# PJLab-ADG/DetZero

Hardware: AMD Instinct MI355X
Metric: LiDAR frames/sec (160k pts, 0.1m voxels) (higher is better)
Workload: dtype f32 as f16 pairs (hi+lo, 22-bit significand; 3 f16 MFMA per product, f32 accumulate)

## Files before the change

detzero_amd/centerpoint.py:

```python
import contextlib
import math
import os

import numpy as np
import torch
import torch.nn as nn

from . import det_modules as cp_modules
from . import iou3d_nms_utils, ops, range_audit as _range_audit
from .lib import DetZeroHipError
from .range_audit import RangeAudit


class CenterPoint(nn.Module):
    def __init__(self, model_cfg, num_class, dataset):
        super().__init__()
        self.model_cfg = model_cfg
        self.num_class = num_class
        self.dataset = dataset
        self.tta = getattr(self.dataset, 'tta', False)
        self.class_names = dataset.class_names
        self.register_buffer('global_step', torch.LongTensor(1).zero_())
        self.second_stage = model_cfg.SECOND_STAGE
        self.module_list = self.build_networks()
# ... 288 lines not shown
        self.split_min = int(os.environ.get('DZ_TUNE_SPLIT_MIN', '12'))
        self._subs = None
        self._way_streams = None
        self.side_key = 0
        self.fork_ok = True
        self.info = dataset_info
        self.mode = mode
        self.dynamic = dynamic
        self.head = model.dense_head
        if len(self.head.class_names_each_head) != 1:
            raise DetZeroHipError('FramePipeline: the batched route packs ONE head\'s detections (the layout of every DetZero config); a '
                                  'multi-head CenterHead runs through the module API (CenterPoint.forward)')
        post = self.head.model_cfg.POST_PROCESSING
        self.k = post.MAX_OBJ_PER_SAMPLE
        self.post_max = post.NMS_CONFIG.NMS_POST_MAXSIZE
        self._streams = {}
        self.level_caps = None
        self._ws = {}
        self.dense_group = int(os.environ.get('DZ_TUNE_DENSE_GROUP', '16'))
        self.last_overflow = None
        self._overflow_acc = None
        self.head_at_candidates = True
        self._partial_head = None

    def _voxelize(self, frames, cid=0):
        info = self.info
        rng = info.point_cloud_range
        nb = len(frames)
        if self.dynamic:
            pb = torch.cat([torch.cat([p.new_full((p.shape[0], 1), float(i)), p], dim=1) for i, p in enumerate(frames)], dim=0)
            return ops.voxelize_dynamic_nosync(pb.contiguous(), rng, info.voxel_size, nb, xy_range_mask=True)
        dev = frames[0].device
        main = torch.cuda.current_stream(dev)
        cap = int(min(info.max_voxels[self.mode], max(max(p.shape[0] for p in frames), 1)))
        c = frames[0].shape[1]
        if nb > 1 and all(p.shape[0] == frames[0].shape[0] for p in frames):
            if isinstance(frames, _StackedFrames):
                pts = frames.tensor.reshape(-1, c)
            else:
                pts = torch.cat(list(frames), dim=0)
            feats, coords, _ = ops.voxelize_hard_mean_batched(pts, nb, rng, info.voxel_size, info.max_points_per_voxel,
                                                              info.max_voxels[self.mode], cap, xy_range_mask=True)
            return feats, coords, None
        feats = torch.empty((nb * cap, c), dtype=torch.float32, device=dev)
        coords = torch.full((nb * cap, 4), -1, dtype=torch.int32, device=dev)
        d_ns = torch.zeros((nb,), dtype=torch.int32, device=dev)
# ... 114 lines not shown
            if self._overflow_acc is None:
                if torch.cuda.is_current_stream_capturing():
                    raise DetZeroHipError('FramePipeline: the overflow counter must exist before graph capture - run calibrate() or '
                                          'one eager pass first (a counter allocated inside a capture is re-zeroed by every replay)')
                self._overflow_acc = torch.zeros((), dtype=torch.int32, device=self.last_overflow.device)
            self._overflow_acc |= self.last_overflow.to(torch.int32)
        return res

    @torch.no_grad()
    def dense_stage(self, res, nb):
        with self._recording():
            return self._dense_stage(res, nb)

    def _dense_stage(self, res, nb):
        m = self.model
        x, lvl = res['encoded']
        sparse = m.backbone3d.math != 0 and m.backbone2d.math == m.backbone3d.math and m.backbone2d.sparse_input_ok(x.shape[1], lvl.shape[0])
        if sparse:
            bev = ops.bev_row_index(lvl, x.shape[0], pad=1)
            run2d = lambda g0, ng: m.backbone2d.run(None, ng, sparse_in=(x, bev[g0:g0 + ng]))
        else:
            bev = ops.sparse_to_bev(x, lvl, x.shape[1], pad=1, math=m.backbone3d.math)
            run2d = lambda g0, ng: m.backbone2d.run(bev[g0:g0 + ng], ng)
        per_frame = bev.shape[1] * bev.shape[2] * max(int(m.backbone2d.num_bev_features), 2 * int(x.shape[1])) * 4
        group = max(1, min(self.dense_group if self.dense_group > 0 else nb, (2 ** 31 - 1) // per_frame))
        at_cand = self.head_at_candidates and self.head.at_candidates_ok()
        self._partial_head = None
        if at_cand:
            self.head.candidate_params()
        if nb <= group:
            with cp_modules.workspace(self._ws):
                concat = run2d(0, nb)
                if not at_cand:
                    return self.head.run_convs(concat, nb)
                shared = self.head.run_shared(concat, nb)
                hd, hh, hw_ = self.head.run_score_head(shared, nb)
                self._partial_head = (hd.data_ptr(), tuple(hd.shape), shared)
                return hd, hh, hw_
        st = {'out': None, 'h': 0, 'w': 0, 'shared': None}

        def head_of_group(concat, g0, ng):
            if at_cand:
                if st['shared'] is None:
                    st['shared'] = cp_modules.bordered_zeros('head.shared_all', (nb,) + tuple(concat.shape[1:3]) + (self.head.plan()['c'],), concat.device)
                hd, st['h'], st['w'] = self.head.run_score_head(self.head.run_shared(concat, ng, out=st['shared'][g0:g0 + ng]), ng)
            else:
                hd, st['h'], st['w'] = self.head.run_convs(concat, ng)
            if st['out'] is None:
                st['out'] = hd.new_empty((nb,) + tuple(hd.shape[1:]))
# ... 256 lines not shown
```

detzero_amd/csrc/conv2d_h.hip:

```cpp
#include "hgemm.h"

namespace dz {

int conv3x3_h_variant(const dz_conv2d_desc &p);
int conv3x3_h_launch(const dz_conv2d_desc &p, int bc, int math, int out_f32, size_t w_bytes, hipStream_t stream);

template <class T, class M, bool OUT_F32, int NS>
__global__ __launch_bounds__(256) void k_conv2d_h(dz_conv2d_desc p, long m_total, unsigned int in_bytes, unsigned int w_bytes) {
    extern __shared__ __attribute__((aligned(16))) unsigned char smem_raw[];
    v4u *const smem = reinterpret_cast<v4u *>(smem_raw);
    __shared__ int in_pix[T::BP];
    __shared__ int out_pix[T::BP];
    __shared__ __attribute__((aligned(16))) float sc_s[T::BC], sh_s[T::BC];

    const int tid = threadIdx.x, lane = tid & 63, wid = tid >> 6;
    const int wp = wid / T::WC, wc = wid % T::WC;
    const int ntn = p.cout_pad / T::BC;
    const int nty = ntn * p.groups;
    const int nwg = gridDim.x, q8 = nwg >> 3, r8 = nwg & 7, xcd = blockIdx.x & 7;
    const int lid = (xcd < r8 ? xcd * (q8 + 1) : r8 * (q8 + 1) + (xcd - r8) * q8) + (blockIdx.x >> 3);
    const int by = lid % nty;
    const int grp = by / ntn;
    const int n0 = (by % ntn) * T::BC;
    const long row0 = (long)(lid / nty) * T::BP;
// ... 157 lines not shown
#pragma unroll
                    for (int e = 0; e < 4; ++e)
                        if (col + e < gcout) o[e] = v[e];
                } else {
                    uint2 hi, lo;
                    split4<M>(v, hi, lo);
                    unsigned char *g = reinterpret_cast<unsigned char *>(p.out) +
                                       ((size_t)op * p.out_cstride + ooff + (col & ~7)) * 4 + (col & 7) * 2;
                    *reinterpret_cast<uint2 *>(g) = hi;
                    *reinterpret_cast<uint2 *>(g + 16) = lo;
                }
            }
        }
    }
}

template <class T, class M, bool OUT_F32, int NS>
static int launch_conv_h(const dz_conv2d_desc &p, size_t w_bytes, hipStream_t stream) {
    const long m_total = (long)p.batch * p.ho * p.wo;
    dim3 grid(ceil_div(m_total, T::BP) * (p.cout_pad / T::BC) * p.groups);
    const size_t in_bytes = (size_t)p.batch * p.in_hp * p.in_wp * p.in_cstride * sizeof(float);
    if (in_bytes >= 0x80000000ull || w_bytes >= 0x80000000ull) {
        set_error("dz_conv2d_forward_split: image of %zu bytes / weights of %zu bytes exceed the 2 GiB buffer-addressing limit", in_bytes, w_bytes);
        return DZ_ERR_UNSUPPORTED;
    }
    static PerDeviceFlags lds_done;
    if (int rc_ = reserve_lds(reinterpret_cast<const void *>(&k_conv2d_h<T, M, OUT_F32, NS>), T::LDS_BYTES, lds_done, "dz_conv2d_forward_split")) return rc_;
    hipLaunchKernelGGL((k_conv2d_h<T, M, OUT_F32, NS>), grid, dim3(256), T::LDS_BYTES, stream, p, m_total, (unsigned int)in_bytes,
                       (unsigned int)w_bytes);
    DZ_LAUNCH_CHECK();
    return DZ_OK;
}

enum ConvHVariant { CH_NONE = 0, CH_128_128, CH_128_64, CH_64_128, CH_64_64, CH_128_32, CH_C3_128, CH_C3_64, CH_C3_32 };
static const char *const kConvHVariantName[] = {"none", "k_conv2d_h<128x128x32>", "k_conv2d_h<128x64x32>", "k_conv2d_h<64x128x32>",
                                                "k_conv2d_h<64x64x32>", "k_conv2d_h<128x32x32>", "k_conv3x3_h<8x32x128>",
                                                "k_conv3x3_h<8x32x64>", "k_conv3x3_h<16x32x32>"};

static ConvHVariant conv2d_h_select(const dz_conv2d_desc &p) {
    if (p.cin % 32 != 0) return CH_NONE;
    const long m_total = (long)p.batch * p.ho * p.wo;
    if (p.cout_pad % 64 != 0) return p.cout_pad % 32 == 0 ? CH_128_32 : CH_NONE;
    struct Cand { ConvHVariant v; int bp, bc; double eff; };
    static const Cand cands[4] = {{CH_128_128, 128, 128, 1.00}, {CH_128_64, 128, 64, 0.90}, {CH_64_128, 64, 128, 0.88}, {CH_64_64, 64, 64, 0.78}};
    const int slots = 512;
    double best = -1.0;
// ... 110 lines not shown
    for (long r0 = 0; r0 < rows; r0 += max_rows) {
        const int n = (int)((rows - r0) < max_rows ? (rows - r0) : max_rows);
        dz_conv2d_desc d = {};
        d.in = x + (size_t)r0 * x_stride; d.out = y + (size_t)(group_max ? r0 / group_rows : r0) * y_stride; d.w = w; d.scale = scale; d.shift = shift;
        d.batch = 1; d.ho = 1; d.wo = n;
        d.in_hp = 1; d.in_wp = n; d.in_cstride = x_stride; d.in_coff = 0; d.cin = cin;
        d.kh = 1; d.kw = 1; d.stride = 1; d.in_off = 0;
        d.out_hp = 1; d.out_wp = n; d.out_cstride = y_stride; d.out_coff = 0;
        d.out_sy = 1; d.out_sx = 1; d.out_dy = 0; d.out_dx = 0;
        d.groups = 1; d.cout_pad = cout_pad; d.g_cout[0] = cout; d.g_ooff[0] = 0; d.relu = relu;
        d.group_shift = group_shift ? group_shift + (size_t)(r0 / group_rows) * cout_pad : nullptr;
        d.group_rows = group_rows;
        d.group_max = group_max ? 1 : 0;
        const int rc = dz_conv2d_forward_split(&d, math, out_f32, stream_);
        if (rc) return rc;
    }
    return DZ_OK;
}

const char *dz_conv2d_variant_split(const dz_conv2d_desc *d, int out_f32) {
    return d ? kConvHVariantName[conv_h_select(*d, out_f32).v] : "none";
}

}
```

detzero_amd/csrc/conv3x3_h.hip:

```cpp
#include "hgemm.h"

namespace dz {

constexpr int C3_TW = 32, C3_KC = 32;
constexpr int C3_ROW_U4 = C3_KC / 4 + 1;
constexpr int C3_PXW = C3_TW + 2;
constexpr int C3_NS = 3;
using v2u = __attribute__((ext_vector_type(2))) unsigned int;

constexpr int C3_NT = 512;
template <int BC>
struct C3Cfg {
    static constexpr int PT = 2;
    static constexpr int WC = BC >= 64 ? 2 : 1;
    static constexpr int WP = C3_NT / 64 / WC;
    static constexpr int TH = WP * PT;
    static constexpr int CT = BC / (32 * WC);
    static constexpr int PXH = TH + 2, PX_ROWS = C3_PXW * PXH, PX_PIECES = PX_ROWS * (C3_KC / 4);
    static constexpr int PXPT = (PX_PIECES + C3_NT - 1) / C3_NT;
    static constexpr int W_PIECES = BC * (C3_KC / 4);
    static constexpr int WPT = (W_PIECES + C3_NT - 1) / C3_NT;
    static constexpr int W_U4 = BC * C3_ROW_U4;
    static constexpr int LDS_MAIN_BYTES = (PX_ROWS * C3_ROW_U4 + 2 * W_U4) * 16;
    static constexpr int SG = 4;
// ... 10 lines not shown
__global__ __launch_bounds__(C3_NT) __attribute__((amdgpu_waves_per_eu(2, 2))) void k_conv3x3_h(dz_conv2d_desc p, int tiles_x, int tiles_y, unsigned int in_bytes,
                                                                                                unsigned int w_bytes, int pair0, int ny) {
    using C = C3Cfg<BC>;
    constexpr int CT = C::CT, PT = C::PT, WPT = C::WPT, C3_PXPT = C::PXPT, WC = C::WC, C3_TH = C::TH,
                  C3_PX_ROWS = C::PX_ROWS, C3_PX_PIECES = C::PX_PIECES;
    extern __shared__ __attribute__((aligned(16))) unsigned char smem_raw[];
    v4u *const px_s = reinterpret_cast<v4u *>(smem_raw);
    v4u *const w_s = px_s + C3_PX_ROWS * C3_ROW_U4;

    const int tid = threadIdx.x, lane = tid & 63, wid = tid >> 6;
    const int wp = wid / WC, wc = wid % WC;
    const int ntn = p.cout_pad / BC, nty = ny;
    const int *const tlist = p.in_tiles;
    const int npx = tlist ? tlist[0] : p.batch * tiles_x * tiles_y;
    const int xcd = blockIdx.x & 7, jloc = blockIdx.x >> 3, nj = gridDim.x >> 3;
    const int grp = (pair0 + jloc % nty) / ntn;
    const int n0 = ((pair0 + jloc % nty) % ntn) * BC;
    const int per_xcd = (npx + 7) >> 3;
    const int band_lo = xcd * per_xcd, band_hi = min(npx, band_lo + per_xcd);
    const int tstep = nj / nty;
    int tile = band_lo + jloc / nty;
    if (tstep == 0 || tile >= band_hi) return;

    const srsrc_t prsrc = make_srsrc(p.in, in_bytes);
    const srsrc_t crsrc = make_srsrc(p.w, w_bytes);
    int x0, y0, b;
    auto tile_id = [&](int t) {
        if (!tlist) return t;
        const int *ptr = tlist + 2 + t;
        int id;
        asm volatile("s_load_dword %0, %1, 0x0\n\ts_waitcnt lgkmcnt(0)" : "=&s"(id) : "s"(ptr) : "memory");
        return id;
    };
    auto tile_origin = [&](int t, int &ox, int &oy, int &ob) {
        ox = (t % tiles_x) * C3_TW;
        oy = ((t / tiles_x) % tiles_y) * C3_TH;
        ob = t / (tiles_x * tiles_y);
    };
    struct TileGeo { unsigned int base; int rows, cols; };
    auto tile_geo = [&](int t) {
        int ox, oy, ob;
        tile_origin(t, ox, oy, ob);
        TileGeo g;
        if constexpr (SPARSE) g.base = (unsigned int)((ob * p.in_hp + oy + p.in_off) * p.in_wp + ox + p.in_off);
        else g.base = (unsigned int)((((long)(ob * p.in_hp + oy + p.in_off) * p.in_wp + ox + p.in_off) * p.in_cstride + p.in_coff + grp * p.cin) * 4);
        g.rows = p.in_hp - (oy + p.in_off);
        g.cols = p.in_wp - (ox + p.in_off);
        return g;
    };
    int id_cur = tile_id(tile), id_next = id_cur;
    TileGeo geo = tile_geo(id_cur), geo_next = geo;
    const int prow = tid / (C3_KC / 4), pq = tid % (C3_KC / 4);
    bool has_next = tile + tstep < band_hi;
    unsigned int cvoff[WPT];
#pragma unroll
    for (int i = 0; i < WPT; ++i) {
        const int idx = tid + i * C3_NT;
        cvoff[i] = idx < C::W_PIECES ? (unsigned int)((((long)grp * 9 * p.cout_pad + n0 + idx / (C3_KC / 4)) * p.cin + (idx % (C3_KC / 4)) * 4) * 4)
                                     : OOB_OFFSET;
    }
    const unsigned int tap_bytes = (unsigned int)((long)p.cout_pad * p.cin * 4);
    const int nk = p.cin / C3_KC;
    const int nchunks = nk * 9;

    v4u wst[C3_NS][WPT];
    v4u pst[C3_PXPT];
    auto issue_w = [&](v4u (&st)[WPT], int chunk) {
        if (chunk >= nchunks) chunk = has_next ? chunk - nchunks : -1;
// ... 31 lines not shown
                if (!((ridx_ok >> i) & 1u)) ridx[i] = v2u{0xFFFFFFFFu, 0xFFFFFFFFu};
            }
        }
    };
    auto issue_px = [&](int kc) {
        if constexpr (SPARSE) {
            const bool cur = kc < nk;
            const bool any = cur || has_next;
            const int kq = cur ? kc : 0, half = nk >> 1;
            const bool z1 = kq >= half;
            const unsigned int sbase = (unsigned int)((kq - (z1 ? half : 0)) * C3_KC * 4 + p.in_coff * 4);
            const unsigned int rowb = (unsigned int)p.in_row_channels * 4u;
#pragma unroll
            for (int i = 0; i < C3_PXPT; ++i) {
                const int ri = (int)(z1 ? ridx[i].y : ridx[i].x);
                const unsigned int off = (any && ri >= 0) ? (unsigned int)ri * rowb + (unsigned int)(pq * 16) : OOB_OFFSET;
                asm volatile("buffer_load_dwordx4 %0, %1, %2, %3 offen" : "=v"(pst[i]) : "v"(off), "s"(prsrc), "s"(sbase));
            }
            return;
        }
        const bool cur = kc < nk;
        const TileGeo g = cur ? geo : geo_next;
        const unsigned int sbase = g.base + (cur ? (unsigned int)(kc * C3_KC * 4) : 0u);
        const bool any = cur || has_next;
        int pr = prow;
        asm volatile("" : "+v"(pr));
#pragma unroll
        for (int i = 0; i < C3_PXPT; ++i) {
            const int r = pr + i * (C3_NT / (C3_KC / 4));
            const int ry = r / C3_PXW, rx = r - ry * C3_PXW;
            const bool ok = any && r < C3_PX_ROWS && ry < g.rows && rx < g.cols;
            const unsigned int off = ok ? (unsigned int)(((ry * p.in_wp + rx) * p.in_cstride + pq * 4) * 4) : OOB_OFFSET;
            asm volatile("buffer_load_dwordx4 %0, %1, %2, %3 offen" : "=v"(pst[i]) : "v"(off), "s"(prsrc), "s"(sbase));
        }
    };
    auto own_w = [&](v4u (&st)[WPT]) {
#pragma unroll
        for (int i = 0; i < WPT; ++i) asm volatile("" : "+v"(st[i]));
    };
    auto store_w = [&](const v4u (&st)[WPT], int buf) {
#pragma unroll
        for (int i = 0; i < WPT; ++i) {
            const int idx = tid + i * C3_NT;
            if (C::W_PIECES % C3_NT == 0 || idx < C::W_PIECES) w_s[buf * C::W_U4 + (idx / (C3_KC / 4)) * C3_ROW_U4 + idx % (C3_KC / 4)] = st[i];
        }
    };
    auto store_px = [&]() {
#pragma unroll
        for (int i = 0; i < C3_PXPT; ++i) {
            asm volatile("" : "+v"(pst[i]));
            const int idx = tid + i * C3_NT;
            if (idx < C3_PX_PIECES) px_s[(idx / (C3_KC / 4)) * C3_ROW_U4 + idx % (C3_KC / 4)] = pst[i];
        }
    };

    f32x16 acc[CT][PT];
// ... 177 lines not shown
        }
    }
    }
    }
    if (!has_next) break;
    tile += tstep;
    id_cur = id_next;
    geo = geo_next;
    has_next = tile + tstep < band_hi;
#pragma unroll
    for (int i = 0; i < CT; ++i)
#pragma unroll
        for (int j = 0; j < PT; ++j)
#pragma unroll
            for (int e = 0; e < 16; ++e) acc[i][j][e] = 0.f;
    }
    asm volatile("s_waitcnt vmcnt(0)");
}

template <int BC, class M, bool OUT_F32, bool SPARSE = false>
static int launch_c3(const dz_conv2d_desc &p, size_t w_bytes, hipStream_t stream) {
    using C = C3Cfg<BC>;
    const int tiles_x = ceil_div(p.wo, C3_TW), tiles_y = ceil_div(p.ho, C::TH);
    const size_t in_bytes = SPARSE ? (size_t)p.in_rows * p.in_row_channels * sizeof(float) : (size_t)p.batch * p.in_hp * p.in_wp * p.in_cstride * sizeof(float);
    if (SPARSE && (size_t)p.batch * p.in_hp * p.in_wp * 8 >= 0x80000000ull) {
        set_error("dz_conv2d_forward_split: row-index image exceeds the 2 GiB buffer-addressing limit");
        return DZ_ERR_UNSUPPORTED;
    }
    if (in_bytes >= 0x80000000ull || w_bytes >= 0x80000000ull) {
        set_error("dz_conv2d_forward_split: image of %zu bytes / weights of %zu bytes exceed the 2 GiB buffer-addressing limit", in_bytes, w_bytes);
        return DZ_ERR_UNSUPPORTED;
    }
    static PerDeviceFlags lds_done;
    if (int rc_ = reserve_lds(reinterpret_cast<const void *>(&k_conv3x3_h<BC, M, OUT_F32, SPARSE>), C::LDS_BYTES, lds_done, "dz_conv2d_forward_split")) return rc_;
    const int nty = p.cout_pad / BC * p.groups;
    const int slots = 32;
    int parts[2][2] = {{0, nty}, {0, 0}};
    const long pair_tiles = (long)p.batch * tiles_x * tiles_y * nty;
    if (slots % nty != 0 && nty < slots && pair_tiles >= 5000) {
        int a = 1;
        while (a * 2 <= nty) a *= 2;
        if (slots % a == 0 && slots % (nty - a) == 0) { parts[0][1] = a; parts[1][0] = a; parts[1][1] = nty - a; }
    }
    for (int k = 0; k < 2 && parts[k][1] > 0; ++k) {
        const int ny = parts[k][1];
        int per_xcd = slots / ny * ny;
        if (per_xcd < ny) per_xcd = ny;
        const long grid = 8L * per_xcd;
        hipLaunchKernelGGL((k_conv3x3_h<BC, M, OUT_F32, SPARSE>), dim3((unsigned int)grid), dim3(C3_NT), C::LDS_BYTES, stream, p, tiles_x,
                           tiles_y, (unsigned int)in_bytes, (unsigned int)w_bytes, parts[k][0], ny);
        DZ_LAUNCH_CHECK();
    }
    return DZ_OK;
// ... 32 lines not shown
```

detzero_amd/det_modules.py:

```python
import contextlib
import os
from functools import partial

import numpy as np
import torch
import torch.nn as nn

from . import ops, range_audit
from .lib import DetZeroHipError
from .range_audit import RangeAudit

PACKED_TABLES = bool(os.environ.get('DZ_TUNE_PACKED_TABLES'))

K3, S1, P1 = (3, 3, 3), (1, 1, 1), (1, 1, 1)


def _inference_only(module):
    if module.training:
        raise DetZeroHipError('%s: only the inference path is implemented on the HIP backend '
                              '(call .eval()); training is out of scope' % type(module).__name__)


def fold_bn(bn, conv_bias=None):
    w = bn.weight.detach().double()
# ... 623 lines not shown
               stride=1, in_off=0, out_cstride, out_coff=0, out_s=1, out_d=(0, 0), groups=1, cout_pad=None,
               g_cout=None, g_ooff=None, ho=None, wo=None, batch=1, math=0, out_f32=False, phase_groups=False, in_rowidx=None,
               in_row_channels=0, in_rows=0, in_tiles=None, w_limb3=None):
    if cout_pad is None:
        cout_pad = w.shape[-2] if math else w.shape[-1]
    desc = dict(
        inp=inp.data_ptr(), out=out.data_ptr(), w=w.data_ptr(),
        scale=scale.data_ptr() if scale is not None else None,
        shift=shift.data_ptr() if shift is not None else None,
        batch=batch, ho=ho, wo=wo, in_hp=in_shape[0], in_wp=in_shape[1], in_cstride=in_cstride, in_coff=in_coff,
        cin=cin, kh=ksize, kw=ksize, stride=stride, in_off=in_off,
        out_hp=out_shape[0], out_wp=out_shape[1], out_cstride=out_cstride, out_coff=out_coff,
        out_sy=out_s, out_sx=out_s, out_dy=out_d[0], out_dx=out_d[1],
        groups=groups, cout_pad=cout_pad,
        g_cout=g_cout if g_cout is not None else [cout_pad], g_ooff=g_ooff if g_ooff is not None else [0],
        relu=1 if relu else 0, phase_groups=1 if phase_groups else 0,
        in_rowidx=in_rowidx.data_ptr() if in_rowidx is not None else None, in_row_channels=int(in_row_channels), in_rows=int(in_rows),
        in_tiles=in_tiles.data_ptr() if in_tiles is not None else None)
    if w_limb3 is not None and not math and ops.conv3x3_limb3_supported(desc):
        desc['w'] = w_limb3().data_ptr()
        ops.conv2d(desc, math=math, out_f32=out_f32, tiles=in_tiles, f32_engine='bf16x3')
        return
    ops.conv2d(desc, math=math, out_f32=out_f32, tiles=in_tiles)


class BaseBEVBackbone(_Cached):

    def __init__(self, model_cfg, input_channels):
        super().__init__()
        self.model_cfg = model_cfg
        layer_nums = list(model_cfg.LAYER_NUMS)
        layer_strides = list(model_cfg.LAYER_STRIDES)
        num_filters = list(model_cfg.NUM_FILTERS)
        upsample_strides = list(model_cfg.UPSAMPLE_STRIDES)
        num_upsample_filters = list(model_cfg.NUM_UPSAMPLE_FILTERS)
        assert len(layer_nums) == len(layer_strides) == len(num_filters) == len(upsample_strides)
        c_in_list = [input_channels, *num_filters[:-1]]
        self.blocks = nn.ModuleList()
        self.deblocks = nn.ModuleList()
        for idx in range(len(layer_nums)):
            cur = [nn.ZeroPad2d(1),
                   nn.Conv2d(c_in_list[idx], num_filters[idx], kernel_size=3, stride=layer_strides[idx], padding=0, bias=False),
                   nn.BatchNorm2d(num_filters[idx], eps=1e-3, momentum=0.01), nn.ReLU()]
            for _ in range(layer_nums[idx]):
                cur.extend([nn.Conv2d(num_filters[idx], num_filters[idx], kernel_size=3, padding=1, bias=False),
                            nn.BatchNorm2d(num_filters[idx], eps=1e-3, momentum=0.01), nn.ReLU()])
# ... 145 lines not shown
            for dx in range(s):
                conv_layer(x, (xh + 2, xw + 2), *self._p(de['phases'][dy][dx], e_mid, e_mid, scale=de['scale'], shift=de['shift']), True, concat,
                           (h + 2, w + 2), cin=de['cin'], in_cstride=xc, ksize=1, stride=1, in_off=1,
                           out_cstride=ctot, out_coff=coff, out_s=s, out_d=(dy + 1, dx + 1), ho=xh, wo=xw,
                           batch=batch, math=self.math)

    def run(self, bev, batch, sparse_in=None):
        plan = self.plan()
        if sparse_in is not None:
            rows, ridx = sparse_in
            dev = rows.device
            h, w = ridx.shape[1] - 2, ridx.shape[2] - 2
        else:
            dev = bev.device
            h, w = bev.shape[1] - 2, bev.shape[2] - 2
        concat = bordered_zeros('bev2d.concat', (batch, h + 2, w + 2, self.num_bev_features), dev)
        x, xh, xw, xc = bev, h, w, (bev.shape[3] if sparse_in is None else 2 * rows.shape[1])
        coff = 0
        for li, lvl in enumerate(plan):
            x, xh, xw, xc = self._level_convs(li, lvl, x, xh, xw, xc, batch, dev, sparse_in=sparse_in if li == 0 else None)
            coff = self._level_deblock(lvl, x, xh, xw, xc, concat, coff, h, w, batch, li)
        return concat

    def grouped_fits(self, nb, h, w):
        plan = self.plan()
        xh, xw, worst = h, w, 0
        for lvl in plan:
            s = lvl['convs'][0]['stride']
            xh, xw = (xh + 2 - 3) // s + 1, (xw + 2 - 3) // s + 1
            worst = max(worst, (xh + 2) * (xw + 2) * lvl['convs'][-1]['cout'] * 4)
        return nb * worst < 2 ** 31

    def run_grouped(self, nb, group, consume, bev=None, sparse_in=None):
        plan = self.plan()
        if sparse_in is not None:
            rows, ridx = sparse_in
            dev = rows.device
            h, w = ridx.shape[1] - 2, ridx.shape[2] - 2
            cin0 = 2 * rows.shape[1]
        else:
            dev = bev.device
            h, w = bev.shape[1] - 2, bev.shape[2] - 2
            cin0 = bev.shape[3]
        l0 = plan[0]
        s0 = l0['convs'][0]['stride']
        h0, w0 = (h + 2 - 3) // s0 + 1, (w + 2 - 3) // s0 + 1
# ... 150 lines not shown
            heads[-1]['score_final'] = {'w': fin['w'][g0:].contiguous(), 'shift': fin['shift'][g0 * 16:].contiguous(),
                                        'shift32': fin['shift32'][g0 * 32:].contiguous(), 'g_cout': g_cout[g0:], 'g_ooff': fin['g_ooff'][g0:]}
        self._plan = {
            'shared': {'w': _conv_weight_taps(sc.weight), 'scale': s_scale, 'shift': s_shift, 'cin': sc.in_channels},
            'heads': heads, 'hidden': heads[0]['hidden'], 'final': heads[0]['final'],
            'c': c, 'order': order,
        }
        return self._plan

    def run_shared(self, concat, batch, out=None):
        p = self.plan()
        hp, wp = concat.shape[1], concat.shape[2]
        c = p['c']
        shared = out if out is not None else bordered_zeros('head.shared', (batch, hp, wp, c), concat.device)
        e = self._e('spatial_features_2d')
        conv_layer(concat, (hp, wp), *self._p(p['shared'], e, e), True, shared, (hp, wp),
                   cin=p['shared']['cin'], in_cstride=concat.shape[3], out_cstride=c, out_d=(1, 1), ho=hp - 2, wo=wp - 2, batch=batch,
                   math=self.math, w_limb3=self._l3(p['shared']))
        audit = range_audit.active()
        if audit is not None:
            audit.probe('dense_head.shared_conv', shared, math=self.math, stage='spatial_features_2d', exp=e)
        return shared

    def run_head(self, shared, batch, index=0):
        p = self.plan()
        hp_ = p['heads'][index]
        dev = shared.device
        hp, wp = shared.shape[1], shared.shape[2]
        h, w = hp - 2, wp - 2
        c = p['c']
        mm = self.math
        hidden = bordered_zeros('head.hidden', (batch, hp, wp, 6 * c), dev)
        e = self._e('spatial_features_2d')
        conv_layer(shared, (hp, wp), *self._p(hp_['hidden'], e, e), True, hidden, (hp, wp),
                   cin=c, in_cstride=c, out_cstride=6 * c, out_d=(1, 1), ho=h, wo=w, batch=batch, math=mm, w_limb3=self._l3(hp_['hidden']))
        head = torch.empty((batch, h * w, 12), dtype=torch.float32, device=dev)
        conv_layer(hidden, (hp, wp), *self._p(hp_['final'], e, 0, scale=None, shift=hp_['final']['shift32' if mm else 'shift']), False, head, (h, w),
                   cin=c, in_cstride=6 * c, out_cstride=12, out_d=(0, 0), groups=6, cout_pad=32 if mm else 16,
                   g_cout=hp_['final']['g_cout'], g_ooff=hp_['final']['g_ooff'], ho=h, wo=w, batch=batch, math=mm, out_f32=True)
        self._audit_head('heads_list.%d' % index, 'hidden', 'final', hidden, head, hp_['final'], e)
        return head, h, w

    def _audit_head(self, prefix, hidden_name, final_name, hidden, head, fin, e):
        audit = range_audit.active()
        if audit is None:
            return
# ... 159 lines not shown
```

detzero_amd/lib.py:

```python
import ctypes
import os

import torch

_HERE = os.path.dirname(os.path.abspath(__file__))
LIB_PATH = os.path.join(_HERE, 'libdetzero_hip.so')


ERR_INVALID, ERR_WORKSPACE, ERR_HIP, ERR_UNSUPPORTED = -1, -2, -3, -4


class DetZeroHipError(RuntimeError):
    pass


c_int, c_float, c_size_t, c_void_p, c_double = ctypes.c_int, ctypes.c_float, ctypes.c_size_t, ctypes.c_void_p, ctypes.c_double
_I3 = c_int * 3
_F3 = c_float * 3
_F6 = c_float * 6
_I8 = c_int * 8


class Conv2dDesc(ctypes.Structure):
    _fields_ = [
# ... 95 lines not shown
    'dz_spconv_x_variant': (ctypes.c_char_p, [c_int, c_int]),
    'dz_spconv_forward_x_f32': (c_int, [c_void_p, c_int, c_int, c_void_p, c_void_p, c_void_p, c_int, c_int, c_void_p, c_void_p, c_void_p, c_void_p,
                                        c_void_p, c_int, c_void_p, c_int, c_void_p]),
    'dz_spconv_x_f32_window_rows': (c_int, [c_int, c_int]),
    'dz_spconv_x_f32_variant': (ctypes.c_char_p, [c_int, c_int]),
    'dz_spconv_forward_x_limb3': (c_int, [c_void_p, c_int, c_int, c_void_p, c_void_p, c_void_p, c_int, c_int, c_void_p, c_void_p, c_void_p, c_void_p,
                                          c_void_p, c_int, c_void_p, c_int, c_void_p]),
    'dz_spconv_x_limb3_window_rows': (c_int, [c_int, c_int]),
    'dz_spconv_x_limb3_variant': (ctypes.c_char_p, [c_int, c_int]),
    'dz_spconv_forward_limb3': (c_int, [c_void_p, c_int, c_int, c_void_p, c_void_p, c_int, c_int, c_void_p, c_void_p, c_void_p, c_void_p,
                                        c_void_p, c_int, c_void_p, c_int, c_void_p]),
    'dz_spconv_limb3_tile_rows': (c_int, [c_int, c_int]),
    'dz_spconv_limb3_variant': (ctypes.c_char_p, [c_int, c_int]),
    'dz_bev_tile_list_words': (c_size_t, [c_int, c_int, c_int]),
    'dz_bev_tile_list': (c_int, [c_void_p, c_int, c_int, c_int, c_int, c_int, c_int, c_void_p, c_void_p, c_void_p]),
    'dz_bev_fill_empty_tiles': (c_int, [c_void_p, c_int, c_int, c_int, c_void_p, c_int, c_int, c_void_p, c_int, c_int, c_int, c_int, c_void_p, c_int, c_void_p]),
    'dz_bev_row_index': (c_int, [c_void_p, c_void_p, c_int, c_int, c_int, c_int, c_int, c_int, c_int, c_void_p, c_void_p]),
    'dz_sparse_to_bev_split': (c_int, [c_void_p, c_void_p, c_void_p, c_int, c_int, c_int, c_int, c_int, c_int, c_void_p,
                                       c_void_p]),
    'dz_sparse_to_bev_split_dense': (c_int, [c_void_p, c_int, c_void_p, c_void_p, c_int, c_int, c_int, c_int, c_int, c_int, c_int, c_void_p,
                                             c_void_p]),
    'dz_conv2d_forward_split': (c_int, [ctypes.POINTER(Conv2dDesc), c_int, c_int, c_void_p]),
    'dz_conv2d_variant_split': (ctypes.c_char_p, [ctypes.POINTER(Conv2dDesc), c_int]),
    'dz_conv3x3_limb3_forward': (c_int, [ctypes.POINTER(Conv2dDesc), c_void_p]),
    'dz_conv3x3_limb3_supported': (c_int, [ctypes.POINTER(Conv2dDesc)]),
    'dz_conv3x3_limb3_variant': (ctypes.c_char_p, [ctypes.POINTER(Conv2dDesc)]),
    'dz_spconv_variant_split': (ctypes.c_char_p, [c_int, c_int]),
    'dz_spconv_variant_split_arm': (ctypes.c_char_p, [c_int, c_int, c_int, c_int, c_size_t]),
    'dz_spconv_variant_split_packed': (ctypes.c_char_p, [c_int, c_int]),
    'dz_xattn_folded_supported': (c_int, [c_int, c_int, c_int]),
    'dz_xattn_folded_workspace_bytes': (ctypes.c_size_t, [c_int, c_int]),
    'dz_xattn_folded': (c_int, [c_void_p] * 6 + [c_int] * 5 + [ctypes.c_float, c_void_p, ctypes.c_size_t, c_void_p, c_void_p]),
    'dz_roi_bev_features': (c_int, [c_void_p, c_int, c_void_p, ctypes.c_long, ctypes.c_long, c_int, c_int, c_int] + [ctypes.c_float] * 4 + [c_int, c_void_p, c_void_p]),
    'dz_linear_splitk_workspace_bytes': (ctypes.c_size_t, [c_int, c_int, c_int]),
    'dz_linear_forward_splitk': (c_int, [c_void_p, c_int, c_int, c_int, c_void_p, c_int, c_int, c_void_p, c_void_p, c_int, c_void_p, c_int, c_int, c_void_p,
                                         ctypes.c_size_t, c_void_p]),
    'dz_mha_core_split': (c_int, [c_void_p, c_void_p, c_void_p, c_void_p, c_int, c_int, c_int, c_int, ctypes.c_float, c_void_p, c_int, c_void_p]),
    'dz_pdv_sa_pool_supported': (c_int, [c_int] * 7),
    'dz_pdv_sa_pool': (c_int, [c_void_p, c_int, c_int, c_void_p, c_void_p, c_int, c_void_p, c_void_p, c_int, c_void_p, c_void_p, c_int,
                               c_void_p, c_int, c_void_p, c_void_p, c_int, c_void_p, c_int, c_void_p, c_void_p, c_int, c_int, c_void_p, c_void_p]),
    'dz_pdv_encoder_front': (c_int, [c_void_p, c_int, c_void_p, c_void_p, ctypes.c_long] + [c_void_p] * 9 + [c_int, c_void_p]),
    'dz_pdv_encoder_back': (c_int, [c_void_p, c_void_p, c_void_p, c_void_p, ctypes.c_long, c_void_p, c_void_p, c_void_p, c_void_p, c_float, c_void_p, c_void_p,
                                    c_void_p, c_void_p, c_void_p, c_void_p, c_float, c_void_p, c_int, c_int, c_void_p]),
    'dz_self_attention_split_supported': (c_int, [c_int, c_int]),
    'dz_self_attention_split': (c_int, [c_void_p, c_void_p, c_void_p, c_int, c_int, c_int, c_void_p, c_int, c_void_p]),
    'dz_pdv_sa_pool_split_supported': (c_int, [c_int] * 7),
# ... 118 lines not shown
```

detzero_amd/ops.py:

```python
import ctypes
import os

import numpy as np
import torch

from . import lib as L


def _dev():
    return torch.device('cuda', torch.cuda.current_device())


def _ws(nbytes):
    return torch.empty((max(int(nbytes), 256),), dtype=torch.uint8, device=_dev())


def grid_size_of(pc_range, voxel_size):
    r = np.asarray(pc_range, dtype=np.float32)
    return np.round((r[3:6] - r[0:3]) / np.array(voxel_size)).astype(np.int64)


def voxelize_hard_nosync(points, pc_range, voxel_size, max_points, max_voxels, xy_range_mask=False):
    lib = L.load()
    L.require_cuda(points)
# ... 610 lines not shown
    out['saturated'], out['nonfinite'], out['elements'] = raw[:, 1], raw[:, 2], raw[:, 3]
    return out


DENSE_F32_ENGINES = ('mfma32', 'bf16x3')


def _conv2d_desc(desc_kwargs):
    d = L.Conv2dDesc()
    for k, v in desc_kwargs.items():
        if k in ('g_cout', 'g_ooff'):
            arr = getattr(d, k)
            for i, e in enumerate(v):
                arr[i] = int(e)
        else:
            setattr(d, k, v)
    return d


def conv3x3_limb3_supported(desc_kwargs):
    return bool(L.load().dz_conv3x3_limb3_supported(ctypes.byref(_conv2d_desc(desc_kwargs))))


def conv2d(desc_kwargs, math=0, out_f32=False, tiles=None, f32_engine=None):
    lib = L.load()
    if f32_engine not in (None,) + DENSE_F32_ENGINES:
        raise L.DetZeroHipError('unknown fp32 dense engine %r (%s)' % (f32_engine, ' | '.join(DENSE_F32_ENGINES)))
    limb3 = f32_engine == 'bf16x3' and not math
    d = _conv2d_desc(desc_kwargs)

    def launch():
        if limb3:
            L.check(lib.dz_conv3x3_limb3_forward(ctypes.byref(d), L.stream()), 'dz_conv3x3_limb3_forward')
        elif math:
            L.check(lib.dz_conv2d_forward_split(ctypes.byref(d), int(math), 1 if out_f32 else 0, L.stream()), 'dz_conv2d_forward_split')
        else:
            L.check(lib.dz_conv2d_forward(ctypes.byref(d), L.stream()), 'dz_conv2d_forward')
    if PROFILER is None:
        launch()
        return
    m = d.batch * d.ho * d.wo
    taps = d.kh * d.kw
    cout = sum(d.g_cout[i] for i in range(d.groups))
    flops = 2.0 * m * taps * d.cin * cout
    nbytes = 4.0 * (m * d.cin * (1 if d.phase_groups else d.groups) + m * cout + taps * d.cin * d.cout_pad * d.groups)
    if tiles is not None:
# ... 449 lines not shown
```

include/detzero_hip.h:

```cpp
#ifndef DETZERO_HIP_H
#define DETZERO_HIP_H

#include <stddef.h>
#include <stdint.h>

#ifdef __cplusplus
extern "C" {
#endif

#define DZ_OK 0
#define DZ_ERR_INVALID (-1)
#define DZ_ERR_WORKSPACE (-2)
#define DZ_ERR_HIP (-3)
#define DZ_ERR_UNSUPPORTED (-4)

const char *dz_version(void);
const char *dz_last_error(void);
int dz_device_cu_count(void);


size_t dz_voxelize_hard_workspace_bytes(int n, int gx, int gy, int gz, int max_points);
int dz_voxelize_hard(const float *points, int n, int c, const float *h_range6, const float *h_vsize3,
                     const int *h_grid3, int xy_range_mask, int max_points, int max_voxels, float *voxels,
                     int *coords_zyx, int *num_points, int *d_num_voxels, void *ws, size_t ws_bytes,
// ... 128 lines not shown
const char *dz_spconv_x_f32_variant(int cin, int cout);
int dz_spconv_forward_x_limb3(const float *in, int in_rows, int cin, const int *nbr_packed, const int *perm, int *windows, int tile_rows,
                              int cap_out, const int *d_m_out, const float *w, const float *scale, const float *shift,
                              const float *residual, int relu, float *out, int cout, void *stream);
int dz_spconv_x_limb3_window_rows(int cin, int cout);
const char *dz_spconv_x_limb3_variant(int cin, int cout);
int dz_spconv_forward_limb3(const float *in, int in_rows, int cin, const int *nbr, const uint32_t *tile_masks, int kvol, int cap_out,
                            const int *d_m_out, const float *w_limb, const float *scale, const float *shift, const float *residual,
                            int relu, float *out, int cout, void *stream);
int dz_spconv_limb3_tile_rows(int cin, int cout);
const char *dz_spconv_limb3_variant(int cin, int cout);
int dz_bev_row_index(const uint32_t *bitmap, const uint32_t *prefix, int batch, int d, int h, int w, int layout, int pad, int feat_rows,
                     int *idx, void *stream);
size_t dz_bev_tile_list_words(int batch, int ho, int wo);
int dz_bev_tile_list(const int *idx, int batch, int hp, int wp, int ho, int wo, int nlists, int *lists, unsigned char *mind_ws, void *stream);
int dz_bev_fill_empty_tiles(const int *list, int batch, int ho, int wo, const float *shift, int relu, int cout, float *out, int out_hp, int out_wp,
                            int out_cstride, int out_coff, const float *zero_resp, int math, void *stream);
int dz_sparse_to_bev_split(const float *feats, const int *coords, const int *d_m, int cap, int c, int d, int h,
                           int w, int pad, float *bev, void *stream);
int dz_sparse_to_bev_split_dense(const float *feats, int feat_rows, const uint32_t *bitmap, const uint32_t *prefix, int batch, int c,
                                 int d, int h, int w, int layout, int pad, float *bev, void *stream);
int dz_conv2d_forward_split(const dz_conv2d_desc *h_desc, int math, int out_f32, void *stream);
const char *dz_conv2d_variant_split(const dz_conv2d_desc *h_desc, int out_f32);
int dz_conv3x3_limb3_forward(const dz_conv2d_desc *h_desc, void *stream);
int dz_conv3x3_limb3_supported(const dz_conv2d_desc *h_desc);
const char *dz_conv3x3_limb3_variant(const dz_conv2d_desc *h_desc);
int dz_linear_forward_split(const float *x, long rows, int cin, int x_stride, const float *w, int cout, int cout_pad, const float *scale,
                            const float *shift, const float *group_shift, int group_rows, int relu, float *y, int y_stride, int math,
                            int out_f32, int group_max, void *stream);
const char *dz_spconv_variant_split(int cin, int cout);
const char *dz_spconv_variant_split_arm(int cin, int cout, int kvol, int has_tile_masks, size_t nbr_bytes);
const char *dz_spconv_variant_split_packed(int cin, int cout);
int dz_xattn_folded_supported(int lq, int e, int heads);
size_t dz_xattn_folded_workspace_bytes(int b, int lk);
int dz_xattn_folded(const float *q, const float *mem, const uint8_t *key_padding_mask, const float *wk_oi, const float *wv_io, const float *bv,
                    int b, int lq, int lk, int e, int heads, float scale, float *workspace, size_t workspace_bytes, float *out, void *stream);
int dz_mlp_chain_forward(const float *x, long rows, const float *wa, const float *sa, const float *ba, const float *group_shift, int ldg, int group_rows,
                         const float *wb, const float *sb, const float *bb, const float *wk, const float *bk, const float *wv, const float *bv,
                         float *mem, float *k, float *v, int math, void *stream);
int dz_pointnet3_forward(const float *x, long rows, const float *w1, const float *s1, const float *b1, const float *w2, const float *s2,
                         const float *b2, const float *w3, const float *s3, const float *b3, int c3, int group_rows, float *tap, float *out,
                         int x_cols_f32, int math, void *stream);

size_t dz_centerhead_decode_workspace_bytes(int batch, int hw, int ncls, int k);
int dz_centerhead_decode(const float *head, int batch, int h, int w, int ncls, int k, float score_thresh,
                         const float *h_limit6, const float *h_range6, const float *h_vsize3, int stride,
// ... 157 lines not shown
```

Before: 1137.

## Size dense frame groups from per-layer buffer limits and rebase conv3x3 per frame

```diff
diff --git a/detzero_amd/centerpoint.py b/detzero_amd/centerpoint.py
--- a/detzero_amd/centerpoint.py
+++ b/detzero_amd/centerpoint.py
@@ -334,6 +334,7 @@
         self._overflow_acc = None
         self.head_at_candidates = True
         self._partial_head = None
+        self._group_fit = {}
 
     def _voxelize(self, frames, cid=0):
         info = self.info
@@ -494,9 +495,18 @@
         else:
             bev = ops.sparse_to_bev(x, lvl, x.shape[1], pad=1, math=m.backbone3d.math)
             run2d = lambda g0, ng: m.backbone2d.run(bev[g0:g0 + ng], ng)
-        per_frame = bev.shape[1] * bev.shape[2] * max(int(m.backbone2d.num_bev_features), 2 * int(x.shape[1])) * 4
-        group = max(1, min(self.dense_group if self.dense_group > 0 else nb, (2 ** 31 - 1) // per_frame))
         at_cand = self.head_at_candidates and self.head.at_candidates_ok()
+        group = min(self.dense_group, nb) if self.dense_group > 0 else nb
+        if group > 1:
+            hp, wp = int(bev.shape[1]), int(bev.shape[2])
+            key = (group, hp, wp, int(x.shape[0]), int(x.shape[1]), sparse, at_cand, int(m.backbone2d.math), int(self.head.math))
+            if key not in self._group_fit:
+                self._group_fit[key] = min(
+                    m.backbone2d.max_frames(group, hp - 2, wp - 2, 2 * int(x.shape[1]) if sparse else int(bev.shape[3]),
+                                            sparse_rows=(int(x.shape[0]), int(x.shape[1])) if sparse else None),
+                    self.head.max_frames(group, hp, wp, int(m.backbone2d.num_bev_features), score_only=at_cand))
+            group = self._group_fit[key]
+        group = max(1, group)
         self._partial_head = None
         if at_cand:
             self.head.candidate_params()
diff --git a/detzero_amd/csrc/conv2d_h.hip b/detzero_amd/csrc/conv2d_h.hip
--- a/detzero_amd/csrc/conv2d_h.hip
+++ b/detzero_amd/csrc/conv2d_h.hip
@@ -203,6 +203,10 @@
     const size_t in_bytes = (size_t)p.batch * p.in_hp * p.in_wp * p.in_cstride * sizeof(float);
     if (in_bytes >= 0x80000000ull || w_bytes >= 0x80000000ull) {
         set_error("dz_conv2d_forward_split: image of %zu bytes / weights of %zu bytes exceed the 2 GiB buffer-addressing limit", in_bytes, w_bytes);
+        return DZ_ERR_UNSUPPORTED;
+    }
+    if ((size_t)p.batch * p.out_hp * p.out_wp >= 0x80000000ull) {
+        set_error("dz_conv2d_forward_split: output image of %zu pixels exceeds the 2^31 pixel index", (size_t)p.batch * p.out_hp * p.out_wp);
         return DZ_ERR_UNSUPPORTED;
     }
     static PerDeviceFlags lds_done;
@@ -359,4 +363,28 @@
     return d ? kConvHVariantName[conv_h_select(*d, out_f32).v] : "none";
 }
 
-}
+int dz_conv2d_max_frames(const dz_conv2d_desc *d, int math, int out_f32) {
+    if (!d || d->batch < 1) return 0;
+    const unsigned long long window = 0x7FFFFFFFull;
+    const unsigned long long frame = (unsigned long long)d->in_hp * d->in_wp * d->in_cstride * sizeof(float);
+    const unsigned long long w_bytes = (unsigned long long)d->groups * d->kh * d->kw * d->cout_pad * d->cin * sizeof(float);
+    if (frame == 0 || frame > window || w_bytes > window) return 0;
+    unsigned long long n = (unsigned long long)d->batch;
+    auto fit = [&](unsigned long long per_frame) { if (per_frame && window / per_frame < n) n = window / per_frame; };
+    if (math != 0) {
+        const ConvHVariant v = conv_h_select(*d, out_f32).v;
+        if (v == CH_NONE) return 0;
+        if (v == CH_C3_128 || v == CH_C3_64 || v == CH_C3_32) {
+            if (d->in_rowidx) {
+                if ((unsigned long long)d->in_rows * d->in_row_channels * sizeof(float) > window) return 0;
+                fit((unsigned long long)d->in_hp * d->in_wp * 8);
+            }
+            return (int)n;
+        }
+    }
+    fit(frame);
+    fit((unsigned long long)d->out_hp * d->out_wp);
+    return (int)n;
+}
+
+}
diff --git a/detzero_amd/csrc/conv3x3_h.hip b/detzero_amd/csrc/conv3x3_h.hip
--- a/detzero_amd/csrc/conv3x3_h.hip
+++ b/detzero_amd/csrc/conv3x3_h.hip
@@ -56,7 +56,8 @@
     int tile = band_lo + jloc / nty;
     if (tstep == 0 || tile >= band_hi) return;
 
-    const srsrc_t prsrc = make_srsrc(p.in, in_bytes);
+    [[maybe_unused]] const srsrc_t prsrc = make_srsrc(p.in, in_bytes);
+    const unsigned int frame_bytes = __builtin_amdgcn_readfirstlane(in_bytes);
     const srsrc_t crsrc = make_srsrc(p.w, w_bytes);
     int x0, y0, b;
     auto tile_id = [&](int t) {
@@ -71,13 +72,19 @@
         oy = ((t / tiles_x) % tiles_y) * C3_TH;
         ob = t / (tiles_x * tiles_y);
     };
-    struct TileGeo { unsigned int base; int rows, cols; };
+    struct TileGeo { unsigned int base; int rows, cols; unsigned int flo, fhi; };
     auto tile_geo = [&](int t) {
         int ox, oy, ob;
         tile_origin(t, ox, oy, ob);
         TileGeo g;
+        g.flo = g.fhi = 0u;
         if constexpr (SPARSE) g.base = (unsigned int)((ob * p.in_hp + oy + p.in_off) * p.in_wp + ox + p.in_off);
-        else g.base = (unsigned int)((((long)(ob * p.in_hp + oy + p.in_off) * p.in_wp + ox + p.in_off) * p.in_cstride + p.in_coff + grp * p.cin) * 4);
+        else {
+            g.base = (unsigned int)((((long)(oy + p.in_off) * p.in_wp + ox + p.in_off) * p.in_cstride + p.in_coff + grp * p.cin) * 4);
+            const unsigned long long fa = (unsigned long long)p.in + (unsigned long long)ob * frame_bytes;
+            g.flo = __builtin_amdgcn_readfirstlane((unsigned int)fa);
+            g.fhi = __builtin_amdgcn_readfirstlane((unsigned int)(fa >> 32) & 0xFFFFu);
+        }
         g.rows = p.in_hp - (oy + p.in_off);
         g.cols = p.in_wp - (ox + p.in_off);
         return g;
@@ -155,6 +162,7 @@
         const bool cur = kc < nk;
         const TileGeo g = cur ? geo : geo_next;
         const unsigned int sbase = g.base + (cur ? (unsigned int)(kc * C3_KC * 4) : 0u);
+        const srsrc_t frsrc = {g.flo, g.fhi, frame_bytes, 0x00020000u};
         const bool any = cur || has_next;
         int pr = prow;
         asm volatile("" : "+v"(pr));
@@ -164,7 +172,7 @@
             const int ry = r / C3_PXW, rx = r - ry * C3_PXW;
             const bool ok = any && r < C3_PX_ROWS && ry < g.rows && rx < g.cols;
             const unsigned int off = ok ? (unsigned int)(((ry * p.in_wp + rx) * p.in_cstride + pq * 4) * 4) : OOB_OFFSET;
-            asm volatile("buffer_load_dwordx4 %0, %1, %2, %3 offen" : "=v"(pst[i]) : "v"(off), "s"(prsrc), "s"(sbase));
+            asm volatile("buffer_load_dwordx4 %0, %1, %2, %3 offen" : "=v"(pst[i]) : "v"(off), "s"(frsrc), "s"(sbase));
         }
     };
     auto own_w = [&](v4u (&st)[WPT]) {
@@ -388,13 +396,14 @@
 static int launch_c3(const dz_conv2d_desc &p, size_t w_bytes, hipStream_t stream) {
     using C = C3Cfg<BC>;
     const int tiles_x = ceil_div(p.wo, C3_TW), tiles_y = ceil_div(p.ho, C::TH);
-    const size_t in_bytes = SPARSE ? (size_t)p.in_rows * p.in_row_channels * sizeof(float) : (size_t)p.batch * p.in_hp * p.in_wp * p.in_cstride * sizeof(float);
+    const size_t in_bytes = SPARSE ? (size_t)p.in_rows * p.in_row_channels * sizeof(float) : (size_t)p.in_hp * p.in_wp * p.in_cstride * sizeof(float);
     if (SPARSE && (size_t)p.batch * p.in_hp * p.in_wp * 8 >= 0x80000000ull) {
         set_error("dz_conv2d_forward_split: row-index image exceeds the 2 GiB buffer-addressing limit");
         return DZ_ERR_UNSUPPORTED;
     }
     if (in_bytes >= 0x80000000ull || w_bytes >= 0x80000000ull) {
-        set_error("dz_conv2d_forward_split: image of %zu bytes / weights of %zu bytes exceed the 2 GiB buffer-addressing limit", in_bytes, w_bytes);
+        set_error("dz_conv2d_forward_split: %s of %zu bytes / weights of %zu bytes exceed the 2 GiB buffer-addressing limit",
+                  SPARSE ? "input rows" : "one frame of the image", in_bytes, w_bytes);
         return DZ_ERR_UNSUPPORTED;
     }
     static PerDeviceFlags lds_done;
diff --git a/detzero_amd/det_modules.py b/detzero_amd/det_modules.py
--- a/detzero_amd/det_modules.py
+++ b/detzero_amd/det_modules.py
@@ -669,6 +669,18 @@
         ops.conv2d(desc, math=math, out_f32=out_f32, tiles=in_tiles, f32_engine='bf16x3')
         return
     ops.conv2d(desc, math=math, out_f32=out_f32, tiles=in_tiles)
+
+
+def conv_layer_max_frames(in_shape, out_shape, *, cin, in_cstride, cout_pad, batch, ho, wo, math, in_coff=0, ksize=3, stride=1, in_off=0,
+                          out_cstride, out_coff=0, out_s=1, out_d=(0, 0), groups=1, out_f32=False, phase_groups=False, sparse=False,
+                          in_row_channels=0, in_rows=0):
+    desc = dict(batch=batch, ho=ho, wo=wo, in_hp=in_shape[0], in_wp=in_shape[1], in_cstride=in_cstride, in_coff=in_coff,
+                cin=cin, kh=ksize, kw=ksize, stride=stride, in_off=in_off,
+                out_hp=out_shape[0], out_wp=out_shape[1], out_cstride=out_cstride, out_coff=out_coff,
+                out_sy=out_s, out_sx=out_s, out_dy=out_d[0], out_dx=out_d[1], groups=groups, cout_pad=cout_pad,
+                g_cout=[cout_pad] * groups, g_ooff=[0] * groups, relu=1, phase_groups=1 if phase_groups else 0,
+                in_rowidx=16 if sparse else None, in_row_channels=int(in_row_channels), in_rows=int(in_rows))
+    return ops.conv2d_max_frames(desc, math=math, out_f32=out_f32)
 
 
 class BaseBEVBackbone(_Cached):
@@ -860,6 +872,27 @@
             coff = self._level_deblock(lvl, x, xh, xw, xc, concat, coff, h, w, batch, li)
         return concat
 
+    def max_frames(self, nb, h, w, cin0, sparse_rows=None):
+        n = nb
+        ctot = self.num_bev_features
+        xh, xw, xc = h, w, cin0
+        for li, lvl in enumerate(self.plan()):
+            for ci, cv in enumerate(lvl['convs']):
+                s = cv['stride']
+                oh, ow = (xh + 2 - 3) // s + 1, (xw + 2 - 3) // s + 1
+                sp = sparse_rows is not None and li == 0 and ci == 0
+                n = min(n, conv_layer_max_frames((xh + 2, xw + 2), (oh + 2, ow + 2), cin=cv['cin'], in_cstride=xc, cout_pad=-(-cv['cout'] // 32) * 32,
+                                                 batch=nb, ho=oh, wo=ow, math=self.math, stride=s, out_cstride=cv['cout'], out_d=(1, 1), sparse=sp,
+                                                 in_rows=sparse_rows[0] if sp else 0, in_row_channels=sparse_rows[1] if sp else 0))
+                xh, xw, xc = oh, ow, cv['cout']
+            de = lvl['de']
+            s = de['s']
+            fused = bool(self.math and 1 < s * s <= 8 and FUSED_DEBLOCK_PHASES)
+            n = min(n, conv_layer_max_frames((xh + 2, xw + 2), (h + 2, w + 2), cin=de['cin'], in_cstride=xc, cout_pad=-(-de['cout'] // 32) * 32, batch=nb,
+                                             ho=xh, wo=xw, math=self.math, ksize=1, in_off=1, out_cstride=ctot, out_s=s, out_d=(1, 1),
+                                             groups=s * s if fused else 1, phase_groups=fused))
+        return n
+
     def grouped_fits(self, nb, h, w):
         plan = self.plan()
         xh, xw, worst = h, w, 0
@@ -1056,6 +1089,18 @@
             audit.probe('dense_head.shared_conv', shared, math=self.math, stage='spatial_features_2d', exp=e)
         return shared
 
+    def max_frames(self, nb, hp, wp, cin_stride, score_only=False, index=0):
+        p = self.plan()
+        c = p['c']
+        ng = 6 - p['heads'][index]['first_score_group'] if score_only else 6
+        h, w = hp - 2, wp - 2
+        n = conv_layer_max_frames((hp, wp), (hp, wp), cin=p['shared']['cin'], in_cstride=cin_stride, cout_pad=-(-c // 32) * 32, batch=nb, ho=h, wo=w,
+                                  math=self.math, out_cstride=c, out_d=(1, 1))
+        n = min(n, conv_layer_max_frames((hp, wp), (hp, wp), cin=c, in_cstride=c, cout_pad=ng * c, batch=nb, ho=h, wo=w, math=self.math,
+                                         out_cstride=ng * c, out_d=(1, 1)))
+        return min(n, conv_layer_max_frames((hp, wp), (h, w), cin=c, in_cstride=ng * c, cout_pad=32 if self.math else 16, batch=nb, ho=h, wo=w,
+                                            math=self.math, out_cstride=12, groups=ng, out_f32=True))
+
     def run_head(self, shared, batch, index=0):
         p = self.plan()
         hp_ = p['heads'][index]
diff --git a/detzero_amd/lib.py b/detzero_amd/lib.py
--- a/detzero_amd/lib.py
+++ b/detzero_amd/lib.py
@@ -141,6 +141,7 @@
                                              c_void_p]),
     'dz_conv2d_forward_split': (c_int, [ctypes.POINTER(Conv2dDesc), c_int, c_int, c_void_p]),
     'dz_conv2d_variant_split': (ctypes.c_char_p, [ctypes.POINTER(Conv2dDesc), c_int]),
+    'dz_conv2d_max_frames': (c_int, [ctypes.POINTER(Conv2dDesc), c_int, c_int]),
     'dz_conv3x3_limb3_forward': (c_int, [ctypes.POINTER(Conv2dDesc), c_void_p]),
     'dz_conv3x3_limb3_supported': (c_int, [ctypes.POINTER(Conv2dDesc)]),
     'dz_conv3x3_limb3_variant': (ctypes.c_char_p, [ctypes.POINTER(Conv2dDesc)]),
diff --git a/detzero_amd/ops.py b/detzero_amd/ops.py
--- a/detzero_amd/ops.py
+++ b/detzero_amd/ops.py
@@ -656,6 +656,11 @@
     return bool(L.load().dz_conv3x3_limb3_supported(ctypes.byref(_conv2d_desc(desc_kwargs))))
 
 
+def conv2d_max_frames(desc_kwargs, math=0, out_f32=False):
+    d = _conv2d_desc(dict(desc_kwargs, inp=desc_kwargs.get('inp') or 16, out=desc_kwargs.get('out') or 16, w=desc_kwargs.get('w') or 16))
+    return int(L.load().dz_conv2d_max_frames(ctypes.byref(d), int(math), 1 if out_f32 else 0))
+
+
 def conv2d(desc_kwargs, math=0, out_f32=False, tiles=None, f32_engine=None):
     lib = L.load()
     if f32_engine not in (None,) + DENSE_F32_ENGINES:
diff --git a/include/detzero_hip.h b/include/detzero_hip.h
--- a/include/detzero_hip.h
+++ b/include/detzero_hip.h
@@ -174,6 +174,7 @@
                                  int d, int h, int w, int layout, int pad, float *bev, void *stream);
 int dz_conv2d_forward_split(const dz_conv2d_desc *h_desc, int math, int out_f32, void *stream);
 const char *dz_conv2d_variant_split(const dz_conv2d_desc *h_desc, int out_f32);
+int dz_conv2d_max_frames(const dz_conv2d_desc *h_desc, int math, int out_f32);
 int dz_conv3x3_limb3_forward(const dz_conv2d_desc *h_desc, void *stream);
 int dz_conv3x3_limb3_supported(const dz_conv2d_desc *h_desc);
 const char *dz_conv3x3_limb3_variant(const dz_conv2d_desc *h_desc);
```

After: 1136. Within noise of the previous version (-0.1%).
